# c-f-h/pyiga

Measured on AMD Instinct MI355X. Metric: assembled elements/sec (3D p=4, 128^3 spans) + HBM-roofline %; 1/2/4/8 GPU, higher is better.
Workload: dtype f64

## Files before the change

### include/igx.h

```cpp
#ifndef IGX_H
#define IGX_H

#include <stddef.h>
#include <stdint.h>

#ifdef __cplusplus
extern "C" {
#endif

#define IGX_VERSION 101
#define IGX_MAX_DIM 3
#define IGX_MAX_DEGREE 15
#define IGX_MAX_SF_DEGREE 7

typedef struct igx_ctx igx_ctx;
typedef struct igx_patch igx_patch;
typedef struct igx_multipatch igx_multipatch;

enum { IGX_MASS = 0, IGX_STIFFNESS = 1,
       IGX_CONVDIFF = 2,
       IGX_FORM = 3 };
enum { IGX_GEO_BSPLINE = 0, IGX_GEO_NURBS = 1, IGX_GEO_JACOBIAN = 2 };
enum { IGX_ALGO_AUTO = 0,
       IGX_ALGO_ENTRYWISE = 1,
// ... 87 lines not shown
int igx_patch_set_form_d(igx_patch *patch, const double *const d_coef[16]);

int igx_patch_set_form_expr(igx_patch *patch, const char *const expr[16], int *cache_hit);
int igx_patch_form_generated(const igx_patch *patch);
int igx_rtc_compile_form(int n, const char *const *expr, const char *arch, char *path_out, int path_len, int *cache_hit);
int igx_rtc_compile_form_fields(int dim, int ncomp, const char *const expr[16], const char *arch, char *path_out, int path_len, int *cache_hit);

int igx_patch_set_pform(igx_patch *patch, int n, const int *masks, const double *const *coef);
int igx_patch_set_basis_orders(igx_patch *patch, const int *slot0, const int *slot1);

int igx_patch_gauss(const igx_patch *patch, int axis, double *nodes, double *weights);

int igx_patch_gauss_slab(const igx_patch *patch, int64_t *g0_lo, int64_t *g0_n);

int igx_patch_last_path(const igx_patch *patch);

int igx_pattern(igx_patch *patch, int32_t *indptr, int32_t *indices);

int igx_assemble(igx_patch *patch, int kind, int algo, double *data_out);
int igx_last_timing(const igx_patch *patch, igx_timing *t);

const double  *igx_d_csr_data(const igx_patch *patch);
const int32_t *igx_d_csr_indices(const igx_patch *patch);
const int32_t *igx_d_csr_indptr(const igx_patch *patch);

int igx_fast_assemble(igx_patch *patch, int kind, double tol, int maxiter, int skipcount, int tolcount, int verbose,
                      double *data_out, int *rank_out, long long *entries_out);
int igx_patch_set_aca_batch(igx_patch *patch, long long max_entries);
int igx_fast_assemble_stats(const igx_patch *patch, long long *requests, long long *entries, int *rank);

// ... 197 lines not shown
```

### pyiga_amd/_lib.py

```python
import ctypes as C
import os
import threading

import numpy as np

_HERE = os.path.dirname(os.path.abspath(__file__))
LIB_PATH = os.environ.get('IGX_LIB') or os.path.join(_HERE, 'libigx.so')

IGX_MASS, IGX_STIFFNESS, IGX_CONVDIFF, IGX_FORM = 0, 1, 2, 3
IGX_GEO_BSPLINE, IGX_GEO_NURBS, IGX_GEO_JACOBIAN = 0, 1, 2
IGX_ALGO_AUTO, IGX_ALGO_ENTRYWISE, IGX_ALGO_SUMFACT = 0, 1, 2
ALGOS = {'auto': IGX_ALGO_AUTO, 'entrywise': IGX_ALGO_ENTRYWISE, 'sumfact': IGX_ALGO_SUMFACT}
KINDS = {'mass': IGX_MASS, 'stiffness': IGX_STIFFNESS, 'convdiff': IGX_CONVDIFF, 'form': IGX_FORM}

_dp = C.POINTER(C.c_double)


class PatchDesc(C.Structure):
    _fields_ = [
        ('dim', C.c_int32), ('p', C.c_int32 * 3), ('kv_len', C.c_int32 * 3), ('kv', _dp * 3),
        ('geo_kind', C.c_int32), ('geo_p', C.c_int32 * 3), ('geo_kv_len', C.c_int32 * 3), ('geo_kv', _dp * 3),
        ('ctrl', _dp), ('jac', _dp),
        ('nqp', C.c_int32), ('gauss_x', _dp), ('gauss_w', _dp),
        ('row0_lo', C.c_int32), ('row0_hi', C.c_int32),
# ... 144 lines not shown
    ('igx_assemble_kron3', C.c_int, [C.c_void_p, C.c_void_p, C.c_int, _dp, _dp, _dp]),
    ('igx_patch_set_coeff_expr', C.c_int, [C.c_void_p, C.c_char_p, C.POINTER(C.c_int)]),
    ('igx_rtc_compile', C.c_int, [C.c_char_p, C.c_char_p, C.c_char_p, C.c_int, C.POINTER(C.c_int)]),
    ('igx_patch_placement', C.c_int, [C.c_void_p, C.POINTER(C.c_int), C.POINTER(C.c_float), C.POINTER(C.c_float)]),
    ('igx_load_vector', C.c_int, [C.c_void_p, _dp, _dp]),
    ('igx_load_vector_jet', C.c_int, [C.c_void_p, _dp * 4, _dp]),
    ('igx_load_vector_jet_expr', C.c_int, [C.c_void_p, C.c_char_p * 4, _dp, C.POINTER(C.c_int)]),
    ('igx_entries_d', C.c_int, [C.c_void_p, C.c_int, C.c_void_p, C.c_size_t, C.c_void_p]),
    ('igx_load_vector_d', C.c_int, [C.c_void_p, C.c_void_p, C.c_void_p]),
    ('igx_fast_assemble', C.c_int, [C.c_void_p, C.c_int, C.c_double, C.c_int, C.c_int, C.c_int, C.c_int, _dp, C.POINTER(C.c_int), C.POINTER(C.c_longlong)]),
    ('igx_patch_set_aca_batch', C.c_int, [C.c_void_p, C.c_longlong]),
    ('igx_fast_assemble_stats', C.c_int, [C.c_void_p, C.POINTER(C.c_longlong), C.POINTER(C.c_longlong), C.POINTER(C.c_int)]),
    ('igx_patch_set_coeff_affine', C.c_int, [C.c_void_p, C.c_double * 4]),
    ('igx_patch_set_form_d', C.c_int, [C.c_void_p, C.c_void_p * 16]),
    ('igx_patch_last_path', C.c_int, [C.c_void_p]),
    ('igx_patch_eval_spline_d', C.c_int, [C.c_void_p, C.c_void_p, C.c_int, C.c_void_p * 4]),
    ('igx_patch_eval_exprs_inputs_d', C.c_int, [C.c_void_p, C.c_int, C.POINTER(C.c_char_p), C.c_int, C.POINTER(C.c_void_p), C.c_void_p, C.POINTER(C.c_int)]),
    ('igx_rtc_compile_exprs_inputs', C.c_int, [C.c_int, C.POINTER(C.c_char_p), C.c_int, C.c_char_p, C.c_char_p, C.c_int, C.POINTER(C.c_int)]),
    ('igx_load_vector_jet_d', C.c_int, [C.c_void_p, C.c_void_p * 4, C.c_void_p]),
    ('igx_patch_gauss_slab', C.c_int, [C.c_void_p, C.POINTER(C.c_int64), C.POINTER(C.c_int64)]),
    ('igx_dev_alloc', C.c_void_p, [C.c_void_p, C.c_size_t]),
    ('igx_dev_free', None, [C.c_void_p, C.c_void_p]),
    ('igx_dev_upload', C.c_int, [C.c_void_p, C.c_void_p, C.c_void_p, C.c_size_t]),
    ('igx_dev_download', C.c_int, [C.c_void_p, C.c_void_p, C.c_void_p, C.c_size_t]),
    ('igx_multipatch_create', C.c_void_p, [C.c_void_p, C.c_int, C.POINTER(C.c_void_p), C.POINTER(C.POINTER(C.c_int32)), C.c_int64]),
    ('igx_multipatch_destroy', None, [C.c_void_p]),
    ('igx_multipatch_get_info', C.c_int, [C.c_void_p, C.POINTER(MultipatchInfo)]),
    ('igx_multipatch_pattern', C.c_int, [C.c_void_p, C.POINTER(C.c_int32), C.POINTER(C.c_int32)]),
    ('igx_multipatch_zero', C.c_int, [C.c_void_p]),
    ('igx_multipatch_scatter_patch', C.c_int, [C.c_void_p, C.c_int, C.c_void_p]),
# ... 165 lines not shown
```

### pyiga_amd/assemblers.py

```python
import os
import ctypes as C
import weakref

import numpy as np
import scipy.sparse

from . import _lib
from . import bspline
from .quadrature import make_tensor_quadrature
from . import geometry

_ENTRY_TRAMPOLINES = []


def _is_spline_geo(geo):
    return hasattr(geo, 'kvs') and hasattr(geo, 'coeffs') and hasattr(geo, 'sdim')


def _is_nurbs(geo):
    from .geometry import NurbsFunc
    return isinstance(geo, NurbsFunc) or type(geo).__name__ == 'NurbsFunc'


class DevicePatch:
# ... 219 lines not shown
        if batch is not None:
            _lib.check(lib.igx_patch_set_aca_batch(self.handle, int(batch)), 'igx_patch_set_aca_batch')
        data = np.empty(self.nnz)
        rank, nent, nreq = C.c_int(0), C.c_longlong(0), C.c_longlong(0)
        _lib.check(lib.igx_fast_assemble(self.handle, _lib.KINDS[kind], float(tol), int(maxiter), int(skipcount), int(tolcount),
                                         int(verbose), _lib.dptr(data), C.byref(rank), C.byref(nent)), 'igx_fast_assemble')
        _lib.check(lib.igx_fast_assemble_stats(self.handle, C.byref(nreq), None, None), 'igx_fast_assemble_stats')
        self.aca_stats = {'rank': rank.value, 'entries': nent.value, 'requests': nreq.value, 'nnz': int(self.nnz)}
        indptr, indices = self.pattern()
        return scipy.sparse.csr_matrix((data, indices, indptr), shape=self.shape)

    def last_path(self):
        bits = _lib.load().igx_patch_last_path(self.handle)
        return {name for bit, name in ((1, 'geoA'), (2, 'fused'), (4, 'mirror'), (8, 'single'), (16, 'kron'), (32, 'both'), (64, 'bf3'), (128, 'twin')) if bits & bit}

    def placement(self):
        n, b, w = C.c_int(0), C.c_float(0), C.c_float(0)
        _lib.check(_lib.load().igx_patch_placement(self.handle, C.byref(n), C.byref(b), C.byref(w)), 'igx_patch_placement')
        return {'tried': n.value, 'best_ms': round(b.value, 4), 'worst_ms': round(w.value, 4)}

    def timing(self):
        t = _lib.Timing()
        _lib.check(_lib.load().igx_last_timing(self.handle, C.byref(t)), 'igx_last_timing')
        return t.as_dict()

    def entries(self, kind, idx):
        idx = np.ascontiguousarray(idx, dtype=np.uintp)
        assert idx.ndim == 2 and idx.shape[1] == 2
        out = np.zeros(idx.shape[0])
        _lib.check(_lib.load().igx_entries(self.handle, _lib.KINDS[kind], idx.ctypes.data_as(C.POINTER(C.c_size_t)),
# ... 759 lines not shown
```

### pyiga_amd/csrc/fused3.hip

```cpp
#include "igx_internal.h"
#include "fused_common.h"
#include <algorithm>
#include <cstdio>
#include <cstdlib>
#include <cstring>
#include <vector>

#ifndef BF3_FIXED_PASS
#define BF3_FIXED_PASS 1
#endif
#ifndef BF3_MASS_AXSYM
#define BF3_MASS_AXSYM 1
#endif
#ifndef BF3_MASS_STW
#define BF3_MASS_STW 1
#endif
#ifndef BF3_MASS_STW_QMAX
#define BF3_MASS_STW_QMAX 3
#endif

namespace igx {

template <int P1, int P2, int Q, int NLG, int NRO, int NCW, int SYM> struct BF3Geom {
    static constexpr int P1_ = P1, P2_ = P2, Q_ = Q;
// ... 348 lines not shown
    cdp V1 = (cdp)A.V1;
    cip fa1 = (cip)A.fa1;
    double acc[P1][P1];
#pragma unroll
    for (int a = 0; a < P1; ++a)
#pragma unroll
        for (int b = 0; b < P1; ++b) acc[a][b] = 0.0;
    __amdgpu_buffer_rsrc_t rsrc[4][NA];
    int urs[4][NA];
    const int voff = g2 * 8;
#pragma unroll
    for (int t1 = 0; t1 < 4; ++t1)
#pragma unroll
        for (int i = 0; i < NA; ++i) {
            urs[t1][i] = A.rs[R.y][t1][i] * 8;
            rsrc[t1][i] = bf2_rsrc(A.sp[R.y][t1][i] + (long long)r0 * A.ss[R.y][t1][i] - (long long)A.gmid_lo * A.rs[R.y][t1][i]);
        }
    auto ld = [&](const int t1, const int i, const int row) {
#ifdef BF3_NOLOAD
        return (double)(row + t1);
#else
        return bf2_buffer_load(rsrc[t1][i], voff, row * urs[t1][i]);
#endif
    };
    static_assert(Q % D == 0, "k_bf3: the prefetch ring must divide the span");
    double kv[D][4][NA];
    {
        const int s = min(s_begin, max(t_sw - 1, 0));
#pragma unroll
        for (int l = 0; l < D; ++l)
#pragma unroll
// ... 620 lines not shown
}

int launch_bf3(hipStream_t st, const igx_patch *pt, const BFInputs &in, double *d_data)
{
    const Axis &AM = *in.mid, &AL = *in.last;
    BFArgs A{};
    int mask = 0, ymax = 0;
    for (int y = 0; y < 4; ++y)
        for (int t1 = 0; t1 < 4; ++t1) {
            const int n = in.slot_n[y][t1];
            if (n > 0) { mask |= 1 << (4 * y + t1); ymax = std::max(ymax, y); }
            if (in.pad_stiff3 && ((BF_MASK_STIFF3 >> (4 * y + t1)) & 1)) { mask |= 1 << (4 * y + t1); ymax = std::max(ymax, y); }
            for (int i = 0; i < 2; ++i) {
                if (i < n) { A.sp[y][t1][i] = in.slot_ptr[y][t1][i]; A.ss[y][t1][i] = in.slice_stride; A.rs[y][t1][i] = AL.G; }
                else { A.sp[y][t1][i] = in.zeros; A.ss[y][t1][i] = 0; A.rs[y][t1][i] = 0; }
            }
        }
    const int ny = ymax == 0 ? 1 : 4;
    A.gmid_lo = in.gmid_lo; A.G2 = AL.G;
    A.V1 = AM.d_V; A.V2 = AL.d_V;
    A.n1 = AM.n; A.N1 = AM.N; A.n2 = AL.n; A.N2 = AL.N;
    A.rp1 = AM.dev.rp; A.rp2 = AL.dev.rp;
    A.fa1 = AM.dev.fa; A.mslo1 = AM.dev.mslo; A.jlo1 = AM.dev.jlo; A.jhi1 = AM.dev.jhi;
    A.pl0 = in.pl0; A.rp0 = in.rp0; A.jlo0 = in.jlo0; A.jhi0 = in.jhi0;
    A.S1 = AM.S; A.S2 = AL.S; A.nnz_off = pt->nnz_off;
    A.data = d_data; A.sym = in.sym;
    A.mid_lo = in.mid_lo; A.mid_hi = in.mid_hi; A.span_hi = in.span_hi;
    A.npairs = in.npairs;
    if (pt->dim == 3) { A.own_lo = pt->r0_lo; A.own_hi = pt->r0_hi; } else { A.own_lo = 0; A.own_hi = 1; }
    const int symk = !in.sym ? 0 : pt->dim == 3 ? ((BF3_MASS_AXSYM && mask == BF_MASK_MASS && ny == 1) ? 3 : 2) : 1;
// ... 18 lines not shown
```

### pyiga_amd/csrc/fused_common.h

```cpp
#pragma once
#include "igx_internal.h"
#include <algorithm>

namespace igx {

typedef const double __attribute__((address_space(4))) *cdp;
typedef const int __attribute__((address_space(4))) *cip;


struct BFRole { int y, shape, f, has[4]; };
constexpr int bf_roles_of_y(int m) { return m == 0 ? 0 : 1; }
constexpr int bf_nroles(int MASK)
{
    return bf_roles_of_y(MASK & 15) + bf_roles_of_y((MASK >> 4) & 15) + bf_roles_of_y((MASK >> 8) & 15) + bf_roles_of_y((MASK >> 12) & 15);
}
constexpr BFRole bf_role_y(int y, int m)
{
    if ((m & 10) == 0) return BFRole{y, 0, 0, {m & 1, 0, (m >> 2) & 1, 0}};
    if ((m & 5) == 0) return BFRole{y, 0, 1, {0, (m >> 1) & 1, 0, (m >> 3) & 1}};
    if ((m & 12) == 0) return BFRole{y, 1, 0, {m & 1, (m >> 1) & 1, 0, 0}};
    if ((m & 3) == 0) return BFRole{y, 1, 1, {0, 0, (m >> 2) & 1, (m >> 3) & 1}};
    return BFRole{y, 2, 0, {m & 1, (m >> 1) & 1, (m >> 2) & 1, (m >> 3) & 1}};
}
constexpr BFRole bf_role(int MASK, int r)
{
    for (int y = 0; y < 4; ++y) {
        const int m = (MASK >> (4 * y)) & 15, n = bf_roles_of_y(m);
        if (r < n) return bf_role_y(y, m);
        r -= n;
    }
    return BFRole{0, 0, 0, {0, 0, 0, 0}};
}
struct BFArgs {
    const double *sp[4][4][2];
    long long ss[4][4][2];
    int rs[4][4][2];
    int gmid_lo;
    int G2;
    const double *V1, *V2;
    int n1, N1, n2, N2;
    const int *rp1, *rp2;
    const int *pl0;
    const int *rp0, *jlo0, *jhi0;
    long long S1, S2, nnz_off;
    double *data;
    int sym;
    int R2, ntiles;
    int mrows, nmchunks;
    unsigned main_blocks;
// ... 172 lines not shown
```

### pyiga_amd/csrc/geoa.hip

```cpp
#include <cstdlib>
#include <cstdio>
#include <algorithm>
#include "geo_device.h"

namespace igx {

constexpr int GA_MAXS = 8;
#ifndef GA_ONEDIV
#define GA_ONEDIV 1
#endif
#ifndef GA_SPREAD
#define GA_SPREAD 0
#endif
#ifndef GA_READBOTH
#define GA_READBOTH 1
#endif
#ifndef GA_DPP
#define GA_DPP 1
#endif
typedef const double __attribute__((address_space(4))) *cdp;
typedef const int __attribute__((address_space(4))) *cip;

struct GeoAArgs {
    GeoView gv;
// ... 9 lines not shown
    int dbg;
#endif
    int field[GA_MAXS], type[GA_MAXS];
    double *out[GA_MAXS];
    int xfield[GA_MAXS], xtype[GA_MAXS];
    const double *coeff;
    int g0_lo, coef_affine;
    double cf[4];
    int soff_ok;
    double pc[16];
    const double *pa[16];
    int pmask, amask, fmask;
    int fslot[16];
    int nsrc[GA_MAXS], sfield[GA_MAXS][4], stype[GA_MAXS][4];
    int nslots;
};
constexpr int GA_NFT = 13;

typedef int int8v __attribute__((ext_vector_type(8)));

#ifdef IGX_ABLATE
#define GA_OFF(bit) (A.dbg & (bit))
#else
#define GA_OFF(bit) false
#endif

#ifdef IGX_GA_STAMP
__device__ unsigned long long g_ga_stamp[2048 * 8 * 6];
#define GA_T(i) do { const unsigned long long n_ = __builtin_amdgcn_s_memtime(); st_[i] += n_ - st_t; st_t = n_; } while (0)
#else
// ... 848 lines not shown
                    if (!plane(j)) break;
            } else {
#pragma unroll 1
                for (int j = 0; j < NS; ++j)
                    if (!plane(j)) break;
            }
            next_batch_barriers(gb + NS, rn);
            rs = rn;
            __syncthreads();
        }
        return;
    }
    if constexpr (DPS) {
        const bool live = w < A.nslots;
        const int t = A.type[w], fi = A.field[w];
        double *const out = A.out[w] + pt;
        const K1Store k1s(A.out[w], pt, tile, A.soff_ok);
        double acc[P][P];
#pragma unroll
        for (int a = 0; a < P; ++a)
#pragma unroll
            for (int b = 0; b < P; ++b) acc[a][b] = 0.0;
        auto products = [&](const int rsl, const int bufn) {
            for (int i = tid; i < NS * 64; i += NT) {
                const int jp = i >> 6, ty = (i >> 4) & 3, m = i & 15;
                const int a = m >= 10 ? 4 : m >= 6 ? 3 : m >= 3 ? 2 : m >= 1 ? 1 : 0, b = m - a * (a + 1) / 2;
                const double x = rec[rsl][jp][6 * (ty >> 1) + a] * rec[rsl][jp][6 * (ty & 1) + b];
                prd_[((bufn * NS + jp) * 4 + ty) * 16 + m] = m < NPR ? x : 0.0;
            }
        };
// ... 32 lines not shown
                GA_T(1);
                if (++l < q) continue;
                const bool write = sp >= own_lo && !GA_OFF(2);
                const int *fr = (const int *)&rec[rs][j][20];
                const int nst = __builtin_amdgcn_readfirstlane(fr[0]), st0 = __builtin_amdgcn_readfirstlane(fr[1]);
                for (int st = st0; st < st0 + nst; ++st) {
                    int pr[P];
                    if (st == st0) {
#pragma unroll
                        for (int a = 0; a < P; ++a) pr[a] = __builtin_amdgcn_readfirstlane(fr[2 + a]);
                    } else {
                        const int8v rec8 = *(const int8v __attribute__((address_space(4))) *)((cip)A.steps + (size_t)st * 8);
#pragma unroll
                        for (int a = 0; a < P; ++a) pr[a] = rec8[a];
                    }
#pragma unroll
                    for (int a = 0; a < P; ++a)
                        if (pr[a] >= 0 && write) k1s.store(out, pr[a], A.stride, acc[a][0]);
#pragma unroll
                    for (int a = 0; a < P - 1; ++a)
#pragma unroll
                        for (int b = 0; b <= a; ++b) acc[a][b] = acc[a + 1][b + 1];
#pragma unroll
                    for (int b = 0; b < P; ++b) acc[P - 1][b] = 0.0;
                }
                l = 0; ++sp;
                GA_T(2);
            }
            GA_T(1);
            next_batch(gb + NS, rn, buf ^ 1);
// ... 207 lines not shown
    if (p0g < 2 || p0g > 3) return false;
    const long long gspans = pt->gax[0].N - pt->gax[0].P + 1;
    return 2 * gspans <= (long long)pt->ax[0].G;
}

bool geoA_form_supported(const igx_patch *pt)
{
    if (pt->dim != 3 || pt->boxed || !pt->knobs.geoa) return false;
    if (pt->geo_kind != IGX_GEO_BSPLINE && pt->geo_kind != IGX_GEO_NURBS) return false;
    const int P = pt->ax[0].P, p0g = pt->gax[0].P;
    if (P < 3 || P > 6 || p0g < 2 || p0g > 3) return false;
    const long long gspans = pt->gax[0].N - pt->gax[0].P + 1;
    return 2 * gspans <= (long long)pt->ax[0].G;
}

int launch_geoA(hipStream_t st, igx_patch *pt, int kind, int nslots, const int *slot_field, const int *slot_type,
                double *const *slot_out, long long slice_stride, int chunk_len, int nchunks, const int *slot_xfield, const int *slot_xtype,
                const GeoAForm *form)
{
    const bool nonsym = kind == IGX_CONVDIFF || (form && !form->sym);
    if (nonsym) {
        if (kind == IGX_CONVDIFF && !pt->coef_affine && !pt->coeff_sampled) { set_error("IGX_CONVDIFF needs igx_patch_set_coeff first"); return IGX_ERR_ARG; }
        if (!pt->d_stepsn) { set_error("internal: flush records of the non-symmetric form are missing"); return IGX_ERR_UNSUPPORTED; }
        if (!pt->d_geoa_tabn) {
            double *tab = nullptr;
            const Axis &A0n = pt->ax[0];
            if (hipMalloc((void **)&tab, (size_t)A0n.G * GA_REC * sizeof(double)) != hipSuccess) { set_error("per-plane table (non-symmetric form): out of device memory"); return IGX_ERR_NOMEM; }
            k_geoa_table<<<dim3((A0n.G + 127) / 128), dim3(128), 0, st>>>(A0n.d_V, A0n.P, pt->gax[0].d_V, pt->gax[0].d_fa, pt->gax[0].P, pt->dev.ax[0].w, A0n.q,
                                                                           pt->stepA_ptr, pt->d_stepsn, A0n.G, tab, nullptr, 1);
            const hipError_t e = hipGetLastError();
            if (e != hipSuccess) { (void)hipFree(tab); set_error("per-plane table (non-symmetric form): %s", hipGetErrorString(e)); return IGX_ERR_HIP; }
            pt->d_geoa_tabn = tab;
        }
// ... 58 lines not shown
    A.w0 = pd.ax[0].w; A.w1 = pd.ax[1].w; A.w2 = d2 ? nullptr : pd.ax[2].w;
    A.nurbs = pt->geo_kind == IGX_GEO_NURBS; A.kind = kind;
    A.G1 = pd.ax[1].G; A.G2 = d2 ? 1 : pd.ax[2].G;
    A.NPL = (long long)A.G1 * A.G2; A.stride = slice_stride;
    A.soff_ok = (long long)(nonsym ? pt->npairs0n : pt->npairs0) * slice_stride * 8 + 1024 < 0x7ffffff0LL ? 1 : 0;
    A.tab = nonsym ? pt->d_geoa_tabn : pt->d_geoa_tab; A.steps = nonsym ? pt->d_stepsn : pt->stepA_rec;
    A.coeff = pt->d_coeff; A.g0_lo = pd.g0_lo; A.coef_affine = pt->coef_affine;
    for (int k = 0; k < 4; ++k) A.cf[k] = pt->coef_c[k];
    A.s_lo = pt->s0_lo; A.s_hi = pt->s0_hi; A.q = A0.q; A.chunk_len = chunk_len;
#ifdef IGX_ABLATE
    { const char *e = getenv("IGX_GEOA_DBG"); A.dbg = e ? atoi(e) : 0; }
#endif
    for (int x = 0; x < nslots; ++x) {
        A.field[x] = slot_field ? slot_field[x] : 0; A.type[x] = slot_type ? slot_type[x] : 0; A.out[x] = slot_out[x];
        A.xfield[x] = slot_xfield ? slot_xfield[x] : -1; A.xtype[x] = slot_xtype ? slot_xtype[x] : 0;
    }
    A.nslots = nslots;
    for (int x = nslots; x < GA_MAXS; ++x) A.out[x] = A.out[0];
    A.ntiles = (int)((A.NPL + 63) / 64);
    dim3 grid((unsigned)((A.ntiles + 7) / 8 * 8), nchunks);
    const int nc = pt->ncomp, p0g = pt->gax[0].P;
    if (d2) {
#define GEOA_2D(PV) case PV: return nslots == 1 ? (p0g == 2 ? launch_geoA_2d<PV, 1, 2>(st, A, nc, grid) : launch_geoA_2d<PV, 1, 3>(st, A, nc, grid)) \
                                                : (p0g == 2 ? launch_geoA_2d<PV, 4, 2>(st, A, nc, grid) : launch_geoA_2d<PV, 4, 3>(st, A, nc, grid))
        switch (A0.P) { GEOA_2D(2); GEOA_2D(3); GEOA_2D(4); GEOA_2D(5); }
#undef GEOA_2D
        set_error("fused geometry + stage A (2D): unsupported degree %d", A0.p);
        return IGX_ERR_UNSUPPORTED;
    }
    if (form) {
        for (int k = 0; k < 16; ++k) { A.pc[k] = form->pc[k]; A.pa[k] = form->pa[k]; A.fslot[k] = form->fslot[k]; }
// ... 38 lines not shown
```

### pyiga_amd/csrc/igx_api.hip

```cpp
#include "igx_internal.h"
#include <algorithm>
#include <cmath>
#include <cstdarg>
#include <cstdio>
#include <cstdlib>
#include <cstring>
#include <new>

namespace igx {

static thread_local char g_err[1024] = "";

void set_error(const char *fmt, ...)
{
    va_list ap;
    va_start(ap, fmt);
    vsnprintf(g_err, sizeof(g_err), fmt, ap);
    va_end(ap);
}

static void gauss_legendre(int n, std::vector<double> &x, std::vector<double> &w)
{
    x.assign(n, 0.0);
    w.assign(n, 0.0);
// ... 340 lines not shown
{
    if (!ctx || !d) { set_error("igx_patch_create: null argument"); return nullptr; }
    const int dim = d->dim;
    if (dim != 2 && dim != 3) { set_error("igx_patch_create: dim must be 2 or 3 (got %d)", dim); return nullptr; }
    if (hipSetDevice(ctx->device) != hipSuccess) { set_error("hipSetDevice failed"); return nullptr; }
    igx_patch *pt = new (std::nothrow) igx_patch();
    if (pt) {
        igx_knobs &k = pt->knobs;
        if (const char *e = getenv("IGX_PATH")) k.path = !strcmp(e, "fused") ? 1 : !strcmp(e, "unfused") ? 2 : !strcmp(e, "single") ? 3 : 0;
        if (const char *e = getenv("IGX_GEOA")) { k.geoa = strcmp(e, "0") != 0; k.geoa_mf = strcmp(e, "mfma") == 0; }
        if (const char *e = getenv("IGX_FINAL")) k.final_sel = !strcmp(e, "q") ? 1 : !strcmp(e, "valu") ? 2 : !strcmp(e, "mfma") ? 3 : 1;
        if (const char *e = getenv("IGX_ENTRIES")) k.entries_thread = !strcmp(e, "thread");
        k.poison = getenv("IGX_DEBUG_POISON") != nullptr;
        if (const char *e = getenv("IGX_BF")) k.bf = atoi(e);
        k.no_twin = getenv("IGX_NO_TWIN") != nullptr;
        if (const char *e = getenv("IGX_PLACEMENT_TRIES")) k.placement_tries = std::max(1, std::min(16, atoi(e)));
        if (const char *e = getenv("IGX_STAGE_EVENTS")) k.stage_events = strcmp(e, "0") != 0;
    }
    if (pt) for (int k = 0; k < 16; ++k) pt->form_slot[k] = -1;
    if (!pt) return nullptr;
    pt->ctx = ctx;
    pt->dim = dim;
    hipStream_t st = ctx->stream;
    int rc = IGX_OK;

    int q = d->nqp;
    if (q <= 0) { q = 0; for (int k = 0; k < dim; ++k) q = std::max(q, d->p[k] + 1); }
    pt->nqp = q;
    std::vector<double> gx, gw;
    if (d->gauss_x && d->gauss_w) { gx.assign(d->gauss_x, d->gauss_x + q); gw.assign(d->gauss_w, d->gauss_w + q); }
// ... 793 lines not shown
    (void)hipEventRecord(pt->ctx->ev[6], st);
    int nl = pt->dim;
    rc = launch_load_vector(st, pt, d_fvals, pt->d_fields, d_out, pt->d_lv_t1, pt->d_lv_t2, -1, 0, &nl);
    (void)hipEventRecord(pt->ctx->ev[7], st);
    if (rc) return rc;
    IGX_HIP(hipStreamSynchronize(st));
    memset(&pt->timing, 0, sizeof(pt->timing));
    (void)hipEventElapsedTime(&pt->timing.total_ms, pt->ctx->ev[6], pt->ctx->ev[7]);
    pt->timing.algo_used = 3;
    pt->timing.n_launches = nl;
    return IGX_OK;
}

int igx_patch_last_path(const igx_patch *pt) { return pt ? pt->last_path : 0; }

int igx_patch_gauss_slab(const igx_patch *pt, int64_t *g0_lo, int64_t *g0_n)
{
    if (!pt) { set_error("igx_patch_gauss_slab: null patch"); return IGX_ERR_ARG; }
    if (g0_lo) *g0_lo = pt->dev.g0_lo;
    if (g0_n) *g0_n = pt->dev.G0_loc;
    return IGX_OK;
}

int igx_load_vector(igx_patch *pt, const double *fvals, double *out)
{
    if (!pt || !fvals || !out) { set_error("igx_load_vector: null argument"); return IGX_ERR_ARG; }
    if (pt->boxed) { set_error("igx_load_vector: the patch holds a span box (batched entries only)"); return IGX_ERR_UNSUPPORTED; }
    IGX_HIP(hipSetDevice(pt->ctx->device));
    hipStream_t st = pt->ctx->stream;
    const PatchDev &pd = pt->dev;
// ... 200 lines not shown
```

### pyiga_amd/csrc/igx_internal.h

```cpp
#pragma once
#include <hip/hip_runtime.h>
#include <stdint.h>
#include <stddef.h>
#include <string>
#include <vector>
#include "igx.h"

namespace igx {

constexpr int MAXP = IGX_MAX_DEGREE + 1;
constexpr int MAX_COMP = 4;

void set_error(const char *fmt, ...);
#define IGX_HIP(call)                                                                   \
    do {                                                                                \
        hipError_t e_ = (call);                                                         \
        if (e_ != hipSuccess) {                                                         \
            igx::set_error("%s:%d: %s -> %s", __FILE__, __LINE__, #call, hipGetErrorString(e_)); \
            return IGX_ERR_HIP;                                                         \
        }                                                                               \
    } while (0)

struct AxisDev {
    int p, P, N, n, q, G;
// ... 67 lines not shown
    int device = 0;
    int ncu = 0;
    hipStream_t stream = nullptr;
    hipEvent_t ev[8] = {};
};

struct igx_knobs {
    int path = 0;
    int geoa = 1;
    int geoa_mf = 0;
    int final_sel = 0;
    int entries_thread = 0;
    int poison = 0;
    int bf = 0;
    int no_twin = 0;
    int placement_tries = 1;
    int stage_events = -1;
};

struct igx_patch;
static inline void stage_event(const igx_patch *pt, int k, hipStream_t st);

struct igx_patch {
    igx_ctx *ctx = nullptr;
    igx_knobs knobs;
    bool basis_default = true;
    bool boxed = false;
    int dim = 0, nqp = 0;
    igx::Axis ax[3];
    int geo_kind = 0, ncomp = 0;
// ... 117 lines not shown
int launch_spline_eval(hipStream_t st, const igx_patch *pt, const double *d_coeffs, int want_grad, double *const d_out[4], double *d_ws);
int launch_form_exprs_inputs(hipStream_t st, igx_patch *pt, int n_expr, const char *const *expr, int m, const double *const *d_in, double *d_out, int *cache_hit);
int rtc_compile_form_inputs(int n_expr, const char *const *expr, int m, const char *arch, char *path_out, int path_len, int *cache_hit);
inline int igx_num_fields(int dim, int kind, int form_n = 0)
{
    return kind == IGX_MASS ? 1 : (kind == IGX_CONVDIFF ? 9 : (kind == IGX_FORM ? form_n : dim * (dim + 1) / 2));
}
constexpr size_t IGX_DUMP_PAD = 1024 * 16 + 16;
inline bool igx_kind_symmetric(int kind) { return kind != IGX_CONVDIFF && kind != IGX_FORM; }
struct BFInputs {
    int pad_stiff3 = 0;
    int tr = 0;
    const Axis *mid, *last;
    int slot_n[4][4];
    const double *slot_ptr[4][4][2];
    long long slice_stride;
    const double *zeros;
    int gmid_lo;
    const int *pl0;
    int npairs;
    const int *rp0, *jlo0, *jhi0;
    int sym, mid_lo, mid_hi;
    int span_hi;
};
struct MirrorInputs {
    const Axis *mid, *last;
    const int *rp0, *jlo0, *jhi0;
    const int *tpairs;
    int ntp;
    int i1_lo, i1_hi;
// ... 6 lines not shown
bool fused3_offsets_fit(int dim, int p0, int p1, int p2, long long S_mid, long long S_last, long long N_last);
bool fused3_degrees(int P1, int P2, int Q, bool sym3d, bool mid_simple);
bool fused3_tr_fits(int p0, int p1, int p2, long long S_mid, long long S_last);
int launch_bf3(hipStream_t st, const igx_patch *pt, const BFInputs &in, double *d_data);
bool geoA_supported(const igx_patch *pt, int kind, int nslots);
struct GeoAForm {
    int sym;
    double pc[16];
    const double *pa[16];
    int pmask;
    int fslot[16];
    int nsrc[8], sfield[8][4], stype[8][4];
};
int launch_geoA(hipStream_t st, igx_patch *pt, int kind, int nslots, const int *slot_field, const int *slot_type,
                double *const *slot_out, long long slice_stride, int chunk_len, int nchunks, const int *slot_xfield = nullptr, const int *slot_xtype = nullptr,
                const GeoAForm *form = nullptr);
bool geoA_form_supported(const igx_patch *pt);

struct Term;
struct XA { int t0, f, slot, key, xt0, xf, alias; };
struct FormPlan {
    bool ok = false, sym = false;
    GeoAForm g;
    int narr = 0;
    int slot_arr[4][4];
    bool mass_only = false;
};
struct Plan {
    enum Chain { FORM_TABLE, SINGLE2D, FUSED2D, STAGES };
    enum Fused { NO_FUSED, BF3, BF2 };
    enum Final { FINAL_VALU, FINAL_Q, FINAL_MFMA };
    int kind = 0;
    bool sym = false, twin = false;
    Chain chain = STAGES;
    bool needs_fields = false;
    bool one_launch = false;
    std::vector<Term> terms;
    std::vector<XA> X;
    std::vector<int> term_x;
    bool merged = false;
    int nX = 0;
    bool geoA = false;
    Fused fused = NO_FUSED;
    int slot_n[4][4] = {}, slot_arr[4][4][2];
    Final fin = FINAL_VALU;
    int mfma_nch = 0;
    FormPlan form;
    Plan();
    ~Plan();
};
void sumfact_plan(const igx_patch *pt, int kind, Plan &pl);
int sumfact_twin_kinds(const igx_patch *tw);
float sumfact_probe_mirror(igx_patch *pt, const Plan &pl, double *buf);
int sumfact_supported(const igx_patch *pt);
int sumfact_prepare(igx_patch *pt);
int sumfact_supports_kind(const igx_patch *pt, int kind);
int sumfact_assemble(igx_patch *pt, const Plan &pl, double *d_data);
}

namespace igx {
struct RowInfo {
    int32_t kstart, len, base, mode;
};
}

struct igx_multipatch {
    igx_ctx *ctx = nullptr;
    int np = 0;
    long long nglobal = 0, nnz = 0;
    bool injective = true;
    long long zero_from = 0;
    long long vzero_from = 0;
// ... 17 lines not shown
```

### pyiga_amd/csrc/sumfact.hip

```cpp
#include "igx_internal.h"
#include "sumfact_stages.h"
#include <algorithm>
#include <cstdio>
#include <cstdlib>
#include <cstring>

namespace igx {

struct LineDesc {
    long long A_d, A_m;
    int bc;
    int flags;
    long long line;
};
struct FinalQArgs {
    const double *V;
    const int *fa, *mslo, *mshi, *jlo, *jhi, *rp;
    int N, G;
    long long nlines;
    const LineDesc *desc;
    long long ndesc;
    int lpw;
    int nchunks;
    int nsuper;
// ... 874 lines not shown
    }
    int nX = 0;
    for (const XA &x : X) nX = std::max(nX, x.slot + 1);
    if (!merged || dim == 2) nX = (int)X.size();
    pl.merged = merged;
    pl.nX = nX;
    pl.geoA = (sym || merged) && geoA_wanted(pt, kind, nX);
    pl.needs_fields = !pl.geoA;

    if (fused && dim == 3) {
        if (merged)
            for (const XA &x : X) add_slot(x.key >> 2, x.key & 3, x.slot);
        else
            for (size_t i = 0; i < terms.size(); ++i) add_slot(kind == IGX_MASS ? 0 : terms[i].t[2], terms[i].t[1], X[term_x[i]].slot);
        pl.fused = fused_kernel();
        if (pl.fused != Plan::NO_FUSED) return;
    }
    const Axis &AL = pt->ax[dim - 1];
    if (pt->knobs.final_sel == 3 && sym && AL.G >= 2 && ldesc_fits(pt)) {
        const int W = 2 * AL.P - 1;
        const int ntile = (AL.N * W + 15) / 16;
        int wmax = 0;
        for (int t = 0; t < ntile; ++t) {
            const int i_first = std::min(AL.N - 1, (t * 16) / W), i_last = std::min(AL.N - 1, (t * 16 + 15) / W);
            wmax = std::max(wmax, (AL.mshi[i_last] - AL.mslo[i_first]) * AL.q);
        }
        pl.mfma_nch = (wmax + 7) / 8;
        if (pl.mfma_nch >= 1 && pl.mfma_nch <= 6) pl.fin = Plan::FINAL_MFMA;
    }
    if (pl.fin != Plan::FINAL_MFMA && pt->knobs.final_sel != 2 && AL.q == AL.P && AL.simple && AL.P <= 6) pl.fin = Plan::FINAL_Q;
// ... 51 lines not shown
        mi.tpairs = pt->d_tpairs; mi.ntp = pt->ntp; mi.i1_lo = i1_lo; mi.i1_hi = i1_hi;
        if (int rc = launch_mirror(st, pt, mi, d_data)) return rc;
        pt->last_path |= IGX_PATH_MIRROR;
        pt->timing.n_launches++;
    }
    stage_event(pt, 4, st);
    return IGX_OK;
}

static BFInputs bf_inputs(const Plan &pl, const double *base, size_t stride)
{
    BFInputs in{};
    for (int y = 0; y < 4; ++y)
        for (int t1 = 0; t1 < 4; ++t1) {
            in.slot_n[y][t1] = pl.slot_n[y][t1];
            for (int i = 0; i < pl.slot_n[y][t1]; ++i) in.slot_ptr[y][t1][i] = base + (size_t)pl.slot_arr[y][t1][i] * stride;
        }
    in.sym = pl.sym ? 1 : 0;
    return in;
}

float sumfact_probe_mirror(igx_patch *pt, const Plan &pl, double *buf)
{
    if (pl.twin || pl.chain != Plan::STAGES || pl.fused != Plan::BF2 || !pl.sym || pt->ntp == 0) return -1.0f;
    hipStream_t st = pt->ctx->stream;
    const Axis &A0 = pt->ax[0];
    MirrorInputs mi{};
    mi.mid = &pt->ax[1]; mi.last = &pt->ax[2]; mi.rp0 = A0.dev.rp; mi.jlo0 = A0.dev.jlo; mi.jhi0 = A0.dev.jhi;
    mi.tpairs = pt->d_tpairs; mi.ntp = pt->ntp; mi.i1_lo = 0; mi.i1_hi = pt->ax[1].N;
    hipEvent_t *ev = pt->ctx->ev;
    float best = -1.0f;
// ... 49 lines not shown
    in.pad_stiff3 = fp.mass_only ? 0 : 1;
    if (!fused3_supported(in)) { set_error("internal: the slots of the form do not fit the fused stage"); return IGX_ERR_UNSUPPORTED; }
    in.slice_stride = NPL; in.gmid_lo = 0; in.pl0 = d_pl0; in.npairs = np0;
    return run_fused(pt, in, sym, d_data, true);
}

static int run_stage0(igx_patch *pt, const Plan &pl, int np0, long long NPL, long long NPLs)
{
    hipStream_t st = pt->ctx->stream;
    const int dim = pt->dim;
    const bool sym = pl.sym;
    const Axis &A0 = pt->ax[0];
    const PatchDev &pd = pt->dev;
    const std::vector<XA> &X = pl.X;
    if (pl.geoA) {
        int sf[8], stp[8], sxf[8], sxt[8];
        double *so[8];
        for (const XA &xa : X) {
            if (xa.alias) continue;
            const int x = pl.merged ? xa.slot : (int)(&xa - X.data());
            sf[x] = xa.f; stp[x] = xa.t0; sxf[x] = xa.xf; sxt[x] = xa.xt0 < 0 ? 0 : xa.xt0;
            so[x] = pt->d_K1 + (size_t)xa.slot * np0 * NPLs;
        }
        const SweepChunks ch = sweep_chunks((NPL + 63) / 64, pt->s0_hi - pt->s0_lo, A0.P, dim == 2 ? geoa2d_min_chunk(A0.P) : 0);
        if (int rc = launch_geoA(st, pt, pl.kind, pl.nX, sf, stp, so, NPLs, ch.len, ch.nchunks, sxf, sxt)) return rc;
        pt->last_path |= IGX_PATH_GEOA;
        pt->timing.n_launches++;
        return IGX_OK;
    }
    const int nF = igx_num_fields(dim, pl.kind, pd.form_n);
    StageAArgs A{};
    int ng = 0;
    const bool one_type = !sym && A0.P >= 5 && A0.q == A0.P;
    for (int f = 0; f < nF; ++f) {
        StageAGroup g{};
        for (size_t x = 0; x < X.size(); ++x)
            if (X[x].f == f && !X[x].alias) {
                if (g.nt == 2) { set_error("internal: more than two stage-A types per field"); return IGX_ERR_UNSUPPORTED; }
                double *o = pt->d_K1 + (size_t)X[x].slot * np0 * NPL;
                if (g.nt == 0) { g.t0 = X[x].t0; g.out0 = o; } else { g.t1 = X[x].t0; g.out1 = o; }
// ... 274 lines not shown
        in.slice_stride = NPLs; in.gmid_lo = 0; in.pl0 = d_pl0; in.npairs = np0;
        return run_fused(pt, in, sym, d_data, pl.fused == Plan::BF3);
    }
    if (pt->is_twin) { set_error("internal: the axis-exchanged twin of a patch left the fused chain"); return IGX_ERR_UNSUPPORTED; }
    if (int rc = ensure_line_descriptors(pt)) return rc;
    FinalArgs F{};
    const double *Kfinal = nullptr;
    int NY = 1;
    if (int rc = run_mid(pt, pl, np0, d_pl0, NPL, F, Kfinal, NY)) return rc;
    stage_event(pt, 3, st);
    if (int rc = run_final(pt, pl, d_pl0, F, Kfinal, NY, d_data)) return rc;
    stage_event(pt, 4, st);
    return IGX_OK;
}

int sumfact_assemble(igx_patch *pt, const Plan &pl, double *d_data)
{
    if (!pl.twin) return run_plan(pt, pl, d_data);
    igx_patch *tw = pt->twin;
    memset(&tw->timing, 0, sizeof(tw->timing));
    tw->last_path = 0;
    const int rc = run_plan(tw, pl, d_data);
    pt->last_path |= tw->last_path | IGX_PATH_TWIN;
    pt->timing.n_launches += tw->timing.n_launches;
    return rc;
}

}
```

Baseline: 174.6 million.

## Skip storing diagonal K1 slices for mirrored stage-A slot pairs in BF3

For symmetric 3D stiffness plans using geoA and the BF3 fused kernel, slots of type 1 and 2 on the same field are paired as mirrors. The geoA sweep no longer writes the diagonal (pr[0]) entries of the higher-indexed mirror slot, and the fused BF3 kernel reads the diagonal row from the partner slot instead. This cuts K1 writes and the related memory traffic, at the cost of extra pointer plumbing and a new invariant between the two kernels. A debug API to poison or check the unused slices is also added, and an env knob can turn the feature off.

```diff
diff --git a/include/igx.h b/include/igx.h
--- a/include/igx.h
+++ b/include/igx.h
@@ -125,6 +125,8 @@
 int igx_patch_gauss_slab(const igx_patch *patch, int64_t *g0_lo, int64_t *g0_n);
 
 int igx_patch_last_path(const igx_patch *patch);
+
+int igx_debug_k1_unused(igx_patch *patch, int kind, int poison);
 
 int igx_pattern(igx_patch *patch, int32_t *indptr, int32_t *indices);
 
diff --git a/pyiga_amd/_lib.py b/pyiga_amd/_lib.py
--- a/pyiga_amd/_lib.py
+++ b/pyiga_amd/_lib.py
@@ -182,6 +182,7 @@
     ('igx_patch_set_coeff_affine', C.c_int, [C.c_void_p, C.c_double * 4]),
     ('igx_patch_set_form_d', C.c_int, [C.c_void_p, C.c_void_p * 16]),
     ('igx_patch_last_path', C.c_int, [C.c_void_p]),
+    ('igx_debug_k1_unused', C.c_int, [C.c_void_p, C.c_int, C.c_int]),
     ('igx_patch_eval_spline_d', C.c_int, [C.c_void_p, C.c_void_p, C.c_int, C.c_void_p * 4]),
     ('igx_patch_eval_exprs_inputs_d', C.c_int, [C.c_void_p, C.c_int, C.POINTER(C.c_char_p), C.c_int, C.POINTER(C.c_void_p), C.c_void_p, C.POINTER(C.c_int)]),
     ('igx_rtc_compile_exprs_inputs', C.c_int, [C.c_int, C.POINTER(C.c_char_p), C.c_int, C.c_char_p, C.c_char_p, C.c_int, C.POINTER(C.c_int)]),
diff --git a/pyiga_amd/assemblers.py b/pyiga_amd/assemblers.py
--- a/pyiga_amd/assemblers.py
+++ b/pyiga_amd/assemblers.py
@@ -257,6 +257,12 @@
         bits = _lib.load().igx_patch_last_path(self.handle)
         return {name for bit, name in ((1, 'geoA'), (2, 'fused'), (4, 'mirror'), (8, 'single'), (16, 'kron'), (32, 'both'), (64, 'bf3'), (128, 'twin')) if bits & bit}
 
+    def debug_k1_unused(self, kind, poison=False):
+        n = _lib.load().igx_debug_k1_unused(self.handle, _lib.KINDS[kind], 1 if poison else 0)
+        if n < 0:
+            _lib.check(n, 'igx_debug_k1_unused')
+        return n
+
     def placement(self):
         n, b, w = C.c_int(0), C.c_float(0), C.c_float(0)
         _lib.check(_lib.load().igx_patch_placement(self.handle, C.byref(n), C.byref(b), C.byref(w)), 'igx_patch_placement')
diff --git a/pyiga_amd/csrc/fused3.hip b/pyiga_amd/csrc/fused3.hip
--- a/pyiga_amd/csrc/fused3.hip
+++ b/pyiga_amd/csrc/fused3.hip
@@ -386,7 +386,8 @@
 #pragma unroll
         for (int i = 0; i < NA; ++i) {
             urs[t1][i] = A.rs[R.y][t1][i] * 8;
-            rsrc[t1][i] = bf2_rsrc(A.sp[R.y][t1][i] + (long long)r0 * A.ss[R.y][t1][i] - (long long)A.gmid_lo * A.rs[R.y][t1][i]);
+            const double *const arr = sc.B->diag0 ? A.spd[R.y][t1][i] : A.sp[R.y][t1][i];
+            rsrc[t1][i] = bf2_rsrc(arr + (long long)r0 * A.ss[R.y][t1][i] - (long long)A.gmid_lo * A.rs[R.y][t1][i]);
         }
     auto ld = [&](const int t1, const int i, const int row) {
 #ifdef BF3_NOLOAD
@@ -1037,6 +1038,7 @@
             for (int i = 0; i < 2; ++i) {
                 if (i < n) { A.sp[y][t1][i] = in.slot_ptr[y][t1][i]; A.ss[y][t1][i] = in.slice_stride; A.rs[y][t1][i] = AL.G; }
                 else { A.sp[y][t1][i] = in.zeros; A.ss[y][t1][i] = 0; A.rs[y][t1][i] = 0; }
+                A.spd[y][t1][i] = (i < n && in.slot_ptr_diag[y][t1][i]) ? in.slot_ptr_diag[y][t1][i] : A.sp[y][t1][i];
             }
         }
     const int ny = ymax == 0 ? 1 : 4;
diff --git a/pyiga_amd/csrc/fused_common.h b/pyiga_amd/csrc/fused_common.h
--- a/pyiga_amd/csrc/fused_common.h
+++ b/pyiga_amd/csrc/fused_common.h
@@ -33,6 +33,7 @@
 }
 struct BFArgs {
     const double *sp[4][4][2];
+    const double *spd[4][4][2];
     long long ss[4][4][2];
     int rs[4][4][2];
     int gmid_lo;
diff --git a/pyiga_amd/csrc/geoa.hip b/pyiga_amd/csrc/geoa.hip
--- a/pyiga_amd/csrc/geoa.hip
+++ b/pyiga_amd/csrc/geoa.hip
@@ -47,6 +47,7 @@
     int fslot[16];
     int nsrc[GA_MAXS], sfield[GA_MAXS][4], stype[GA_MAXS][4];
     int nslots;
+    int nodiag[GA_MAXS];
 };
 constexpr int GA_NFT = 13;
 
@@ -925,6 +926,7 @@
     if constexpr (DPS) {
         const bool live = w < A.nslots;
         const int t = A.type[w], fi = A.field[w];
+        const bool nodiag = A.nodiag[w] != 0;
         double *const out = A.out[w] + pt;
         const K1Store k1s(A.out[w], pt, tile, A.soff_ok);
         double acc[P][P];
@@ -987,6 +989,7 @@
 #pragma unroll
                         for (int a = 0; a < P; ++a) pr[a] = rec8[a];
                     }
+                    if (nodiag) pr[0] = -1;
 #pragma unroll
                     for (int a = 0; a < P; ++a)
                         if (pr[a] >= 0 && write) k1s.store(out, pr[a], A.stride, acc[a][0]);
@@ -1224,9 +1227,15 @@
     return 2 * gspans <= (long long)pt->ax[0].G;
 }
 
+bool geoA_diag_couples(const igx_patch *pt)
+{
+    const int P = pt->ax[0].P;
+    return GA_DPP && pt->knobs.diag_couples && pt->dim == 3 && P * (P + 1) / 2 <= 16 && !pt->knobs.geoa_mf;
+}
+
 int launch_geoA(hipStream_t st, igx_patch *pt, int kind, int nslots, const int *slot_field, const int *slot_type,
                 double *const *slot_out, long long slice_stride, int chunk_len, int nchunks, const int *slot_xfield, const int *slot_xtype,
-                const GeoAForm *form)
+                const GeoAForm *form, const int *slot_nodiag)
 {
     const bool nonsym = kind == IGX_CONVDIFF || (form && !form->sym);
     if (nonsym) {
@@ -1315,7 +1324,9 @@
     for (int x = 0; x < nslots; ++x) {
         A.field[x] = slot_field ? slot_field[x] : 0; A.type[x] = slot_type ? slot_type[x] : 0; A.out[x] = slot_out[x];
         A.xfield[x] = slot_xfield ? slot_xfield[x] : -1; A.xtype[x] = slot_xtype ? slot_xtype[x] : 0;
-    }
+        A.nodiag[x] = slot_nodiag ? slot_nodiag[x] : 0;
+    }
+    if (slot_nodiag && (nonsym || form || d2 || !geoA_diag_couples(pt))) { set_error("internal: diagonal pairs left out of a sweep that does not reproduce them"); return IGX_ERR_UNSUPPORTED; }
     A.nslots = nslots;
     for (int x = nslots; x < GA_MAXS; ++x) A.out[x] = A.out[0];
     A.ntiles = (int)((A.NPL + 63) / 64);
diff --git a/pyiga_amd/csrc/igx_api.hip b/pyiga_amd/csrc/igx_api.hip
--- a/pyiga_amd/csrc/igx_api.hip
+++ b/pyiga_amd/csrc/igx_api.hip
@@ -378,6 +378,7 @@
         k.poison = getenv("IGX_DEBUG_POISON") != nullptr;
         if (const char *e = getenv("IGX_BF")) k.bf = atoi(e);
         k.no_twin = getenv("IGX_NO_TWIN") != nullptr;
+        if (const char *e = getenv("IGX_DIAG_COUPLES")) k.diag_couples = strcmp(e, "0") != 0;
         if (const char *e = getenv("IGX_PLACEMENT_TRIES")) k.placement_tries = std::max(1, std::min(16, atoi(e)));
         if (const char *e = getenv("IGX_STAGE_EVENTS")) k.stage_events = strcmp(e, "0") != 0;
     }
@@ -1201,6 +1202,14 @@
 
 int igx_patch_last_path(const igx_patch *pt) { return pt ? pt->last_path : 0; }
 
+int igx_debug_k1_unused(igx_patch *pt, int kind, int poison)
+{
+    if (!pt || !sumfact_supports_kind(pt, kind)) { set_error("igx_debug_k1_unused: bad argument"); return -IGX_ERR_ARG; }
+    if (!pt->sumfact_ok || hipSetDevice(pt->ctx->device) != hipSuccess) return 0;
+    const int n = sumfact_debug_k1_unused(pt, kind, poison != 0);
+    return n;
+}
+
 int igx_patch_gauss_slab(const igx_patch *pt, int64_t *g0_lo, int64_t *g0_n)
 {
     if (!pt) { set_error("igx_patch_gauss_slab: null patch"); return IGX_ERR_ARG; }
diff --git a/pyiga_amd/csrc/igx_internal.h b/pyiga_amd/csrc/igx_internal.h
--- a/pyiga_amd/csrc/igx_internal.h
+++ b/pyiga_amd/csrc/igx_internal.h
@@ -105,6 +105,7 @@
     int poison = 0;
     int bf = 0;
     int no_twin = 0;
+    int diag_couples = 1;
     int placement_tries = 1;
     int stage_events = -1;
 };
@@ -252,6 +253,7 @@
     const Axis *mid, *last;
     int slot_n[4][4];
     const double *slot_ptr[4][4][2];
+    const double *slot_ptr_diag[4][4][2];
     long long slice_stride;
     const double *zeros;
     int gmid_lo;
@@ -288,8 +290,9 @@
 };
 int launch_geoA(hipStream_t st, igx_patch *pt, int kind, int nslots, const int *slot_field, const int *slot_type,
                 double *const *slot_out, long long slice_stride, int chunk_len, int nchunks, const int *slot_xfield = nullptr, const int *slot_xtype = nullptr,
-                const GeoAForm *form = nullptr);
+                const GeoAForm *form = nullptr, const int *slot_nodiag = nullptr);
 bool geoA_form_supported(const igx_patch *pt);
+bool geoA_diag_couples(const igx_patch *pt);
 
 struct Term;
 struct XA { int t0, f, slot, key, xt0, xf, alias; };
@@ -317,6 +320,7 @@
     bool geoA = false;
     Fused fused = NO_FUSED;
     int slot_n[4][4] = {}, slot_arr[4][4][2];
+    int mirror[8] = {-1, -1, -1, -1, -1, -1, -1, -1};
     Final fin = FINAL_VALU;
     int mfma_nch = 0;
     FormPlan form;
@@ -330,6 +334,7 @@
 int sumfact_prepare(igx_patch *pt);
 int sumfact_supports_kind(const igx_patch *pt, int kind);
 int sumfact_assemble(igx_patch *pt, const Plan &pl, double *d_data);
+int sumfact_debug_k1_unused(igx_patch *pt, int kind, bool poison);
 }
 
 namespace igx {
diff --git a/pyiga_amd/csrc/sumfact.hip b/pyiga_amd/csrc/sumfact.hip
--- a/pyiga_amd/csrc/sumfact.hip
+++ b/pyiga_amd/csrc/sumfact.hip
@@ -912,6 +912,11 @@
         else
             for (size_t i = 0; i < terms.size(); ++i) add_slot(kind == IGX_MASS ? 0 : terms[i].t[2], terms[i].t[1], X[term_x[i]].slot);
         pl.fused = fused_kernel();
+        if (pl.fused == Plan::BF3 && sym && !merged && pl.geoA && nX <= 8 && geoA_diag_couples(pt)) {
+            for (size_t a = 0; a < X.size(); ++a)
+                for (size_t b = 0; b < X.size(); ++b)
+                    if (X[a].f == X[b].f && X[a].t0 == 1 && X[b].t0 == 2) { pl.mirror[X[a].slot] = X[b].slot; pl.mirror[X[b].slot] = X[a].slot; }
+        }
         if (pl.fused != Plan::NO_FUSED) return;
     }
     const Axis &AL = pt->ax[dim - 1];
@@ -993,7 +998,11 @@
     for (int y = 0; y < 4; ++y)
         for (int t1 = 0; t1 < 4; ++t1) {
             in.slot_n[y][t1] = pl.slot_n[y][t1];
-            for (int i = 0; i < pl.slot_n[y][t1]; ++i) in.slot_ptr[y][t1][i] = base + (size_t)pl.slot_arr[y][t1][i] * stride;
+            for (int i = 0; i < pl.slot_n[y][t1]; ++i) {
+                const int a = pl.slot_arr[y][t1][i], m = (a >= 0 && a < 8) ? pl.mirror[a] : -1;
+                in.slot_ptr[y][t1][i] = base + (size_t)a * stride;
+                if (m >= 0 && m < a) in.slot_ptr_diag[y][t1][i] = base + (size_t)m * stride;
+            }
         }
     in.sym = pl.sym ? 1 : 0;
     return in;
@@ -1073,16 +1082,19 @@
     const PatchDev &pd = pt->dev;
     const std::vector<XA> &X = pl.X;
     if (pl.geoA) {
-        int sf[8], stp[8], sxf[8], sxt[8];
+        int sf[8], stp[8], sxf[8], sxt[8], snd[8];
         double *so[8];
+        bool any_nd = false;
         for (const XA &xa : X) {
             if (xa.alias) continue;
             const int x = pl.merged ? xa.slot : (int)(&xa - X.data());
             sf[x] = xa.f; stp[x] = xa.t0; sxf[x] = xa.xf; sxt[x] = xa.xt0 < 0 ? 0 : xa.xt0;
             so[x] = pt->d_K1 + (size_t)xa.slot * np0 * NPLs;
+            snd[x] = (pl.mirror[xa.slot] >= 0 && pl.mirror[xa.slot] < xa.slot) ? 1 : 0;
+            any_nd |= snd[x] != 0;
         }
         const SweepChunks ch = sweep_chunks((NPL + 63) / 64, pt->s0_hi - pt->s0_lo, A0.P, dim == 2 ? geoa2d_min_chunk(A0.P) : 0);
-        if (int rc = launch_geoA(st, pt, pl.kind, pl.nX, sf, stp, so, NPLs, ch.len, ch.nchunks, sxf, sxt)) return rc;
+        if (int rc = launch_geoA(st, pt, pl.kind, pl.nX, sf, stp, so, NPLs, ch.len, ch.nchunks, sxf, sxt, nullptr, any_nd ? snd : nullptr)) return rc;
         pt->last_path |= IGX_PATH_GEOA;
         pt->timing.n_launches++;
         return IGX_OK;
@@ -1387,6 +1399,37 @@
     return IGX_OK;
 }
 
+int sumfact_debug_k1_unused(igx_patch *pt, int kind, bool poison)
+{
+    Plan pl;
+    sumfact_plan(pt, kind, pl);
+    igx_patch *p = pl.twin ? pt->twin : pt;
+    if (!p || pl.chain != Plan::STAGES || pl.fused != Plan::BF3 || !pl.geoA || !pl.sym || p->dim != 3 || !p->d_K1) return 0;
+    const size_t np0 = (size_t)p->npairs0, NPL = (size_t)p->ax[1].G * p->ax[2].G;
+    if (p->K1_cap < (size_t)pl.nX * np0 * NPL || p->h_pl0.size() < 2 * np0) return 0;
+    hipStream_t st = p->ctx->stream;
+    if (hipStreamSynchronize(st) != hipSuccess) { set_error("igx_debug_k1_unused: synchronize failed"); return -IGX_ERR_HIP; }
+    std::vector<double> first;
+    int n = 0;
+    for (int x = 0; x < pl.nX && x < 8; ++x) {
+        if (pl.mirror[x] < 0 || pl.mirror[x] >= x) continue;
+        for (size_t r0 = 0; r0 < np0; ++r0) {
+            if (p->h_pl0[2 * r0] != p->h_pl0[2 * r0 + 1]) continue;
+            double *slice = p->d_K1 + ((size_t)x * np0 + r0) * NPL;
+            if (poison) {
+                if (hipMemsetAsync(slice, 0xff, NPL * sizeof(double), st) != hipSuccess) { set_error("igx_debug_k1_unused: memset failed"); return -IGX_ERR_HIP; }
+                ++n;
+            } else {
+                first.push_back(0.0);
+                if (hipMemcpy(&first.back(), slice, sizeof(double), hipMemcpyDeviceToHost) != hipSuccess) { set_error("igx_debug_k1_unused: copy failed"); return -IGX_ERR_HIP; }
+                if (first.back() != first.back()) ++n;
+            }
+        }
+    }
+    if (hipStreamSynchronize(st) != hipSuccess) { set_error("igx_debug_k1_unused: synchronize failed"); return -IGX_ERR_HIP; }
+    return n;
+}
+
 int sumfact_assemble(igx_patch *pt, const Plan &pl, double *d_data)
 {
     if (!pl.twin) return run_plan(pt, pl, d_data);
```

After: 171.2 million. 0.981x the previous value.
